# iamycy/golf

Hardware: AMD Instinct MI355X
Metric: audio samples/sec (24 kHz) GOLF-ss synth, batch=32x2 s, 4 batches in flight (higher is better)
Workload: dtype f32

## Files before the change

### golf_amd/csrc/glottal_osc.hip

```cpp
#include "common.h"
#include "device_common.h"
#include "lpc_p1f.h"
#include <algorithm>

namespace golf {

struct OscGeom {
    int P;
    int N;
    int hop_t;
    int nint;
    int ntile;
    int pre_stride;
    size_t off_cw, off_ttot, off_pre, off_part, off_bfr, off_bf4, off_look, total;
};
#define OSC_SCAN_TILE 1024

static void osc_geom(int B, int Tp, int phase_hop, int Fw, int w_hop, int os, OscGeom* g) {
    g->P = phase_hop * os;
    g->N = g->P > 1 ? (Tp - 1) * g->P + 1 : Tp;
    g->hop_t = w_hop * os;
    g->nint = (int)ceil_div(g->N, g->hop_t);
    size_t o = 0;
    g->ntile = (int)ceil_div(Tp, OSC_SCAN_TILE);
// ... 1640 lines not shown
    if (amp) expect = std::min(expect, amp_hop > 1 ? (Fa - 1) * amp_hop + 1 : Fa);
    if (tscale) expect = std::min(expect, ts_hop > 1 ? (Fs - 1) * ts_hop + 1 : Fs);
    if (hp.poff) expect = (int)std::min<int64_t>(expect, (int64_t)(hp.Fo - 1) * hp.po_hop + 1);
    if (Tout != expect) return fail(GOLF_EINVAL, "%s: Tout=%d, expected %d", who, Tout, expect);
    if (amp && dyn_lds && (size_t)(g.nrows + 1) * H * sizeof(float) > 60 * 1024)
        return fail(GOLF_EUNSUPPORTED, "%s: amplitude hop %d too fine for %d harmonics (LDS staging); pass amplitudes "
                    "at a coarser hop or fold them into tscale/hscale", who, amp_hop, H);
    if (dyn_lds && HARM_STATIC_LDS + dyn_lds > HARM_LDS_LIMIT) {
        if (amp)
            return fail(GOLF_EUNSUPPORTED, "%s: amplitude hop %d too fine for %d harmonics%s (LDS staging: %zu bytes, limit "
                        "%zu); pass amplitudes at a coarser hop or fold them into tscale/hscale", who, amp_hop, H,
                        hp.phi0 ? " with initial_phase" : "", HARM_STATIC_LDS + dyn_lds, HARM_LDS_LIMIT);
        return fail(GOLF_EUNSUPPORTED, "%s: %d harmonics%s too many for the LDS staging (%zu bytes, limit %zu)", who, H,
                    hp.phi0 ? " with initial_phase" : "", HARM_STATIC_LDS + dyn_lds, HARM_LDS_LIMIT);
    }
    return GOLF_OK;
}

struct SrcArgs {
    const float* phase; int64_t phase_stride; OscLook look; u64* Ttot; const float* wsel; int Fw; const float* table; int n_tab, L,
        lshift, Tp, hop_t; const float* Bf4; float* out; int64_t out_stride; int Tout, dmin, nrows; const float* addend;
    int64_t addend_stride; int Tadd, B, ntile;
};
struct MapArgs { const float* a; float* PhiT; int F, M, hop, L, NP, nq; float* pmax; unsigned* fixcnt; int B; float* Phi; };
#ifdef SRCMAPS_TIMING
__device__ unsigned long long g_srcmaps_rt[4 * 2048];
extern "C" int golf_debug_srcmaps_rt(unsigned long long* host_out, int n) {
    return (int)hipMemcpyFromSymbol(host_out, HIP_SYMBOL(g_srcmaps_rt), sizeof(unsigned long long) * (size_t)n);
}
#define SRCMAPS_RT(i, v) do { if ((threadIdx.x & 63) == 0 && blockIdx.x < 2048 && (threadIdx.x == 0 || (i) == 3)) g_srcmaps_rt[4 * blockIdx.x + (i)] = (v); } while (0)
#else
#define SRCMAPS_RT(i, v) do { } while (0)
#endif
template <int EE, int KS, int W, int NT>
__global__ __launch_bounds__(512) __attribute__((amdgpu_waves_per_eu(3, 3))) void source_maps_kernel(SrcArgs o, MapArgs m,
                                                                                                     int nblk_f) {
    extern __shared__ __attribute__((aligned(16))) float smem[];
    SRCMAPS_RT(0, __builtin_amdgcn_s_memrealtime());
    SRCMAPS_RT(2, ((unsigned long long)__builtin_amdgcn_s_getreg(4 | (31 << 11))) | ((unsigned long long)(__builtin_amdgcn_s_getreg(20 | (3 << 11)) & 15) << 32));
    if ((int)blockIdx.x < nblk_f) {
        if (threadIdx.x >= 64 * P1F_WPB) return;
#ifndef SRCMAPS_PRIO_MAPS
#define SRCMAPS_PRIO_MAPS 0
#endif
        __builtin_amdgcn_s_setprio(SRCMAPS_PRIO_MAPS);
        p1f_body<W, NT>(m.a, m.PhiT, m.F, m.M, m.hop, m.L, m.NP, m.nq, smem, (int)blockIdx.x, m.pmax, m.fixcnt, m.B, m.Phi);
        SRCMAPS_RT(1, __builtin_amdgcn_s_memrealtime());
    } else {
#ifndef SRCMAPS_PRIO_OSC
#define SRCMAPS_PRIO_OSC 1
#endif
        const int u = (int)blockIdx.x - nblk_f;
#ifdef SRCMAPS_HI_UNITS
        if (u < SRCMAPS_HI_UNITS) __builtin_amdgcn_s_setprio(3); else __builtin_amdgcn_s_setprio(SRCMAPS_PRIO_OSC);
#else
        __builtin_amdgcn_s_setprio(SRCMAPS_PRIO_OSC);
#endif
        const int tile = u / o.B, b = u - tile * o.B;
        osc_fused2_tile<EE, KS, 2048, 512>(o.phase, o.phase_stride, o.look, o.Ttot, o.wsel, o.Fw, o.table, o.n_tab, o.L, o.lshift,
                                           o.Tp, o.hop_t, o.Bf4, o.out, o.out_stride, o.Tout, o.dmin, o.nrows, o.addend,
                                           o.addend_stride, o.Tadd, smem, tile, b, o.ntile);
        SRCMAPS_RT(1, __builtin_amdgcn_s_memrealtime());
    }
}

}

using namespace golf;

// ... 169 lines not shown
                                              addend_stride, Tadd, tap_frags))
            return rc;
        return golf_ltv_allpole_transitions_f32(a, B, T, F, M, hop, ss_ws, ss_ws_bytes, ss_flags, stream);
    }
    hipStream_t st = (hipStream_t)stream;
    const float* Bf4 = tap_frags ? (const float*)tap_frags + kTapFragFloats : (const float*)((char*)osc_ws + g.off_bf4);
    if (!tap_frags) {
        hipLaunchKernelGGL(osc_tap_frags_kernel, dim3(4), dim3(256), 0, st, taps, K, f2.dmin, f2.dmax, f2.KS,
                           (float*)((char*)osc_ws + g.off_bf4), (float*)((char*)osc_ws + g.off_bfr));
        GOLF_LAUNCH_CHECK();
    }
    SrcArgs o;
    o.phase = phase; o.phase_stride = phase_stride;
    o.look.gen = (unsigned*)((char*)osc_ws + g.off_look);
    o.look.ent = (unsigned long long*)((char*)osc_ws + g.off_look + 256 * ceil_div((size_t)B * 4, 256));
    o.Ttot = (u64*)((char*)osc_ws + g.off_ttot);
    o.wsel = wsel; o.Fw = Fw; o.table = table; o.n_tab = n_tab; o.L = L; o.lshift = f2.lshift; o.Tp = Tp; o.hop_t = g.hop_t;
    o.Bf4 = Bf4; o.out = out; o.out_stride = out_stride; o.Tout = Tout; o.dmin = f2.dmin; o.nrows = f2.nrows;
    o.addend = addend; o.addend_stride = addend_stride; o.Tadd = Tadd; o.B = B; o.ntile = f2.ntile_f;
    char* sw = (char*)ss_ws;
    MapArgs m;
    m.a = a; m.PhiT = (float*)(sw + p.off_phiT); m.F = F; m.M = M; m.hop = hop; m.L = p.L; m.NP = p.NP; m.nq = B * p.NP;
    m.pmax = (float*)(sw + p.off_pmax); m.fixcnt = (unsigned*)(sw + p.off_fixcnt); m.B = B;
    m.Phi = (ss_flags & GOLF_SS_TRAINING) ? (float*)(sw + p.off_phi) : (float*)nullptr;
    const int nblk_f = (int)ceil_div(m.nq, P1fGeom<24, 22, 2>::CPW * P1F_WPB);
    const unsigned grid = (unsigned)(nblk_f + B * f2.ntile_f);
#define GOLF_SRC_MAPS(EE, KSV)                                                                                        \
    do {                                                                                                              \
        static const hipError_t lds_attr = hipFuncSetAttribute(                                                       \
            (const void*)source_maps_kernel<EE, KSV, 24, 22>, hipFuncAttributeMaxDynamicSharedMemorySize, 160 * 1024); \
        if (lds_attr != hipSuccess)                                                                                   \
            return fail((int)lds_attr, "source_transitions: cannot raise the dynamic LDS limit: %s",                  \
                        hipGetErrorString(lds_attr));                                                                 \
        hipLaunchKernelGGL((source_maps_kernel<EE, KSV, 24, 22>), dim3(grid), dim3(512), f2.lds, st, o, m, nblk_f);   \
    } while (0)
    if (f2.KS == 12) { if (equal_energy & 1) GOLF_SRC_MAPS(1, 12); else GOLF_SRC_MAPS(0, 12); }
    else             { if (equal_energy & 1) GOLF_SRC_MAPS(1, 16); else GOLF_SRC_MAPS(0, 16); }
#undef GOLF_SRC_MAPS
    GOLF_LAUNCH_CHECK();
    return GOLF_OK;
}

extern "C" int golf_glottal_osc_bwd_wsel_f32(const float* g_out, int64_t g_out_stride, const float* phase,
                                             int64_t phase_stride, int Tp, int phase_hop, const float* wsel, int Fw,
                                             int w_hop, const float* table, int n_tab, int L, int os, int equal_energy,
                                             const float* taps, int K, float* g_wsel, int B, int Tout, void* ws,
// ... 574 lines not shown
```

### golf_amd/csrc/lpc_p1f.h

```cpp
#pragma once
#include "device_common.h"

namespace golf {

typedef float f32x2 __attribute__((ext_vector_type(2)));

constexpr int P1F_WPB = 4;
template <int W, int NT, int NR = 2>
struct P1fGeom {
    static constexpr int KT = 2 * NR;
    static constexpr int NG = (NT + KT - 1) / KT;
    static constexpr int CPW = 64 / NG;
    static constexpr int WAVE_TILE = 64;
    static constexpr int TILE_FLOATS = P1F_WPB * WAVE_TILE;
};
template <int W, int NT, int NR = 2>
__device__ __forceinline__ void p1f_body(const float* __restrict__ a, float* __restrict__ PhiT, int F, int M, int hop,
                                         int L, int NP, int nq, float* __restrict__ tile_all, int blk_id,
                                         float* __restrict__ pmax, unsigned* __restrict__ fixcnt = nullptr, int B = 0,
                                         float* __restrict__ Phi = nullptr) {
    using G = P1fGeom<W, NT, NR>;
    constexpr int KT = G::KT, NG = G::NG, CPW = G::CPW;
    constexpr int NP2 = NT / 2;
    const int lane = threadIdx.x & 63;
    const int wv = __builtin_amdgcn_readfirstlane(threadIdx.x >> 6);
    float* tile = tile_all + wv * G::WAVE_TILE;
    const int cl = lane / NG, grp = lane - cl * NG;
    const int q0 = (blk_id * P1F_WPB + wv) * CPW;
    if (fixcnt && blk_id == 0 && wv == 0)
        for (int e = lane; e < 5 * B + 1; e += 64) fixcnt[e] = 0u;
    if (q0 >= nq) return;
    const int q = q0 + cl;
    const bool live = cl < CPW && q < nq;
    const int jb = KT * grp;
    const int qq = live ? q : (nq - 1);
    const int b = qq / NP, c = qq - b * NP;
    f32x2 h[NR][W];
#pragma unroll
    for (int r = 0; r < NR; ++r)
#pragma unroll
        for (int k = 0; k < W; ++k) {
            const int j = W - 1 - k, j0 = jb + 2 * r;
            h[r][k] = f32x2{(j == j0 && j0 < M) ? 1.f : 0.f, (j == j0 + 1 && j0 + 1 < M) ? 1.f : 0.f};
        }
    f32x2 a0p[NP2], ddp[NP2];
    const float inv_hop = 1.0f / (float)hop;
    int fcur = -1;
    const int nblk = L / W;
    for (int blk = 0; blk < nblk; ++blk) {
        const int t0 = c * L + blk * W;
        const int f = t0 / hop;
        if (f != fcur) {
            fcur = f;
// ... 107 lines not shown
```

### golf_amd/csrc/lpc_ss.hip

```cpp
#include "common.h"
#include "device_common.h"
#include "lpc_p1f.h"
#include <cstdlib>
#include <type_traits>

namespace golf {

static float phi_guard() {
    static const float v = [] { const char* e = getenv("GOLF_SS_PHI_GUARD"); return e ? (float)atof(e) : 30.f; }();
    return v;
}
static float phi_guard2() {
    static const float v = [] { const char* e = getenv("GOLF_SS_PHI_GUARD2"); return e ? (float)atof(e) : 8.f; }();
    return v;
}
static float group_log2_guard() {
    static const float v = [] { const char* e = getenv("GOLF_SS_GROUP_LOG2"); return e ? (float)atof(e) : 96.f; }();
    return v;
}
static int hot_all_16ths() {
    static const int v = [] { const char* e = getenv("GOLF_SS_HOT_ALL_16THS"); return e ? atoi(e) : 16; }();
    return v;
}
static int hot_count() {
// ... 531 lines not shown
            }
            const R cf0 = cfq[(NT - 1) % PD];
            const int sp = (s - 1 + W) % W;
#pragma unroll
            for (int r = 0; r < KT; ++r) h[r][s] = __builtin_elementwise_fma(-cf0, h[r][sp], -(ra[r] + rb[r]));
            __builtin_amdgcn_sched_barrier(0);
        }
    }
#pragma unroll
    for (int r = 0; r < KT; ++r) {
        const int j = jb + r;
        if (j < NT) {
            float* o = Phi + ((size_t)q * NT + j) * W;
#pragma unroll
            for (int i = 0; i < W; ++i) o[i] = (i < M && j < M) ? (float)h[r][W - 1 - i] : 0.f;
        }
    }
}

template <int W, int NT, int NR = 2>
__global__ __launch_bounds__(64 * P1F_WPB) void lpc_p1f_kernel(const float* __restrict__ a, float* __restrict__ PhiT,
                                                               int F, int M, int hop, int L, int NP, int nq,
                                                               float* __restrict__ pmax, unsigned* __restrict__ fixcnt,
                                                               int B, float* __restrict__ Phi) {
    __shared__ __attribute__((aligned(16))) float tile_all[P1fGeom<W, NT, NR>::TILE_FLOATS];
    p1f_body<W, NT, NR>(a, PhiT, F, M, hop, L, NP, nq, tile_all, blockIdx.x, pmax, fixcnt, B, Phi);
}

template <int W, int NT>
__device__ __forceinline__ void p1z_units(const float* __restrict__ ex, int64_t ex_stride,
                                          const float* __restrict__ gain, const float* __restrict__ a,
                                          float* __restrict__ z, int T, int F, int M, int hop, int L, int NP, int ncg,
                                          int B, int upw, int zblk, float (*xt)[Tile<W, 16>::SIZE]) {
    const int wv = __builtin_amdgcn_readfirstlane(threadIdx.x >> 6);
    light_wave_priority();
    for (int u = 0; u < upw; ++u) {
        const int unit = (zblk * 4 + wv) * upw + u;
        if (unit >= ncg * B) return;
        fwdq_body<W, NT, 0>(ex, ex_stride, gain, a, nullptr, z, 0, T, F, M, hop, L, NP, NP, nullptr, xt[wv], nullptr,
                            unit / ncg, unit - (unit / ncg) * ncg, threadIdx.x & 63);
        wave_lds_fence();
    }
}

template <int W, int NT>
__global__ __launch_bounds__(64 * P1F_WPB) void lpc_p1fz_kernel(const float* __restrict__ ex, int64_t ex_stride,
                                                                const float* __restrict__ gain,
                                                                const float* __restrict__ a, float* __restrict__ z,
                                                                float* __restrict__ PhiT, int T, int F, int M, int hop,
                                                                int L, int NP, int nq, int nblk_f, int ncg, int B,
                                                                int upw, float* __restrict__ pmax,
                                                                unsigned* __restrict__ fixcnt, float* __restrict__ Phi) {
    using TL = Tile<W, 16>;
    __shared__ __attribute__((aligned(16))) float tile_all[P1fGeom<W, NT>::TILE_FLOATS];
    __shared__ float xt[P1F_WPB][TL::SIZE];
    if ((int)blockIdx.x < nblk_f) {
        p1f_body<W, NT>(a, PhiT, F, M, hop, L, NP, nq, tile_all, blockIdx.x, pmax, fixcnt, B, Phi);
    } else {
        p1z_units<W, NT>(ex, ex_stride, gain, a, z, T, F, M, hop, L, NP, ncg, B, upw, (int)blockIdx.x - nblk_f, xt);
    }
}

template <int W, int NT, int KT>
__global__ __launch_bounds__(256) void lpc_p1hz_kernel(const float* __restrict__ ex, int64_t ex_stride,
                                                       const float* __restrict__ gain, const float* __restrict__ a,
                                                       float* __restrict__ z, float* __restrict__ Phi,
                                                       float* __restrict__ PhiT, int T, int F, int M, int hop, int L,
                                                       int NP, int nq, int nblk_h, int ncg, int B, int upw) {
    using TL = Tile<W, 16>;
    __shared__ float xt[4][TL::SIZE];
    if ((int)blockIdx.x < nblk_h) {
        constexpr int NG = (NT + KT - 1) / KT;
        const int nqb = (nq + 63) / 64;
        const int unit = blockIdx.x * 4 + __builtin_amdgcn_readfirstlane(threadIdx.x >> 6);
        const int qblk = unit / NG, grp = unit - qblk * NG;
        if (qblk >= nqb) return;
        p1_hom_body<W, NT, KT, double>(qblk, grp, a, Phi, PhiT, F, M, hop, L, NP, nq);
    } else {
        p1z_units<W, NT>(ex, ex_stride, gain, a, z, T, F, M, hop, L, NP, ncg, B, upw, (int)blockIdx.x - nblk_h, xt);
    }
}

template <int W, int NT>
__global__ __launch_bounds__(256) void lpc_transpose_kernel(const float* __restrict__ Phi, float* __restrict__ PhiT,
                                                            int nq, float* __restrict__ pmax,
                                                            unsigned* __restrict__ fixcnt, int B) {
    __shared__ float t[4][NT * (W + 1)];
    const int wv = threadIdx.x >> 6, lane = threadIdx.x & 63;
    if (fixcnt && blockIdx.x == 0)
        for (int e = threadIdx.x; e < 5 * B + 1; e += 256) fixcnt[e] = 0u;
    const int q = blockIdx.x * 4 + wv;
    if (q >= nq) return;
    const float* src = Phi + (size_t)q * NT * W;
    float* dst = PhiT + (size_t)q * NT * W;
    float* tt = t[wv];
    unsigned mx = 0u;
    for (int e = lane; e < NT * W; e += 64) {
        const int j = e / W, i = e - j * W;
        const float v = src[e];
        tt[j * (W + 1) + i] = v;
        mx = max(mx, __float_as_uint(fabsf(v)));
    }
    if (pmax) {
#pragma unroll
        for (int off = 32; off >= 1; off >>= 1) mx = max(mx, (unsigned)__shfl_xor((int)mx, off));
        if (lane == 0) pmax[q] = __uint_as_float(mx);
    }
    __builtin_amdgcn_s_waitcnt(0);
    __builtin_amdgcn_wave_barrier();
    for (int e = lane; e < NT * W; e += 64) {
        const int i = e / W, j = e - i * W;
        dst[e] = (j < NT) ? tt[j * (W + 1) + i] : 0.f;
    }
// ... 40 lines not shown
        if (g3 > 0.f && hot16 > 0 && n * 16u >= (unsigned)NP * (unsigned)hot16) d.t3 = true;
        else if (d.t2) d.nhot = n;
    }
    if (d.t3) d.nhot = (unsigned)NP;
    return d;
}

template <int CTRL>
__device__ __forceinline__ double dppd(double v) {
    const long long x = __builtin_bit_cast(long long, v);
    const unsigned lo = (unsigned)__builtin_amdgcn_update_dpp(0, (int)(unsigned)x, CTRL, 0xF, 0xF, true);
    const unsigned hi = (unsigned)__builtin_amdgcn_update_dpp(0, (int)(unsigned)(x >> 32), CTRL, 0xF, 0xF, true);
    return __builtin_bit_cast(double, ((long long)hi << 32) | (long long)lo);
}
struct FixArgs {
    const float* a;
    float* PhiT;
    float* Phi;
    double* Phi64;
    const float* pmax;
    unsigned* tier;
    unsigned* status;
    unsigned* fixcnt;
    int F, M, hop, L, NP, B;
    float g1, g2, g3, glog;
    int hot16, hotn;
    int accurate;
};

constexpr int kHotListMax = 512;
template <typename T> __device__ __forceinline__ void st_through(T* p, T v) {
    __hip_atomic_store(p, v, __ATOMIC_RELAXED, __HIP_MEMORY_SCOPE_AGENT);
}
template <int W, int NT>
__device__ __forceinline__ void fixup_wave(const FixArgs& fa, int b, bool writes_tier, unsigned short* __restrict__ hotlist) {
    constexpr int TPL = quad_tpl(W, NT);
    const int lane = threadIdx.x & 63;
    const int row = lane >> 2, r = lane & 3;
    const int NP = fa.NP, M = fa.M, F = fa.F, hop = fa.hop, L = fa.L;
    const float* pm = fa.pmax + (size_t)b * NP;
    const UttTier d = utterance_tier(pm, NP, lane, fa.g1, fa.g2, fa.g3, fa.accurate, fa.glog, fa.hot16, fa.hotn);
    if (writes_tier && lane == 0) {
        fa.tier[2 * b] = d.t3 ? kTierPrecise : (d.t2 ? kTierHot : 0u);
        fa.tier[2 * b + 1] = d.nhot;
    }
    if (d.nhot == 0u) return;
    const bool listed = NP <= kHotListMax;
    if (listed) {
        int base = 0;
        for (int c0 = 0; c0 < NP; c0 += 64) {
            const int c = c0 + lane;
            const bool h = c < NP && (d.t3 || !(fabsf(pm[c < NP ? c : 0]) <= fa.g2));
            const unsigned long long m = __builtin_amdgcn_ballot_w64(h);
            const int pre = __builtin_amdgcn_mbcnt_hi((unsigned)(m >> 32), __builtin_amdgcn_mbcnt_lo((unsigned)m, 0u));
            if (h) hotlist[base + pre] = (unsigned short)c;
            base += __builtin_popcountll(m);
        }
        wave_lds_fence();
    }
    const int total = (listed ? (int)d.nhot : NP) * NT;
    unsigned done = 0u;
    for (;;) {
        int k0 = 0;
        if (lane == 0) k0 = (int)atomicAdd(fa.fixcnt + fa.B + b, 16u);
        k0 = __builtin_amdgcn_readfirstlane(k0);
        if (k0 >= total) break;
        const int k = k0 + row;
        const bool live = k < total;
        done += (unsigned)((total - k0 < 16) ? total - k0 : 16);
        const int h = live ? k / NT : 0, j = live ? k - h * NT : 0;
        const int c = listed ? (int)hotlist[h] : h;
        const bool hot = live && (listed || d.t3 || !(fabsf(pm[c]) <= fa.g2));
        if (!hot) continue;
        const size_t q = (size_t)b * NP + c;
        double* o64 = fa.Phi64 + (q * NT + j) * W;
        if (d.t3)
            for (int i = 4 * TPL + r; i < W; i += 4) st_through(o64 + i, 0.0);
        if (j >= M) {
            if (d.t3) {
#pragma unroll
                for (int kk = 0; kk < TPL; ++kk) st_through(o64 + r * TPL + kk, 0.0);
            }
            continue;
// ... 58 lines not shown
            if (fa.Phi) {
                float* o2 = fa.Phi + (q * NT + j) * W;
#pragma unroll
                for (int kk = 0; kk < TPL; ++kk) {
                    const int i = r * TPL + kk;
                    if (i < W) st_through(o2 + i, i < M ? (float)w[TPL - 1 - kk] : 0.f);
                }
            }
        }
        if (d.t3) {
#pragma unroll
            for (int kk = 0; kk < TPL; ++kk) {
                const int i = r * TPL + kk;
                st_through(o64 + i, i < M ? w[TPL - 1 - kk] : 0.0);
            }
        }
    }
    if (!done) return;
    __builtin_amdgcn_fence(__ATOMIC_RELEASE, "workgroup");
    __builtin_amdgcn_s_waitcnt(0x0F70);
    if (lane == 0 && done) atomicAdd(fa.fixcnt + b, done);
}

__device__ __forceinline__ void wait_for_fixup(const FixArgs& fa, int b, unsigned nhot, int NT) {
    const unsigned expected = (fa.NP <= kHotListMax ? nhot : (unsigned)fa.NP) * (unsigned)NT;
    unsigned it = 0u;
    while (__hip_atomic_load(fa.fixcnt + b, __ATOMIC_RELAXED, __HIP_MEMORY_SCOPE_AGENT) < expected) {
        __builtin_amdgcn_s_sleep(8);
        if (++it > (1u << 16)) {
            if ((threadIdx.x & 63) == 0) atomicOr(fa.fixcnt + 2 * fa.B, 1u);
            break;
        }
    }
    __builtin_amdgcn_fence(__ATOMIC_ACQUIRE, "agent");
}

template <int W, int NT>
__global__ __launch_bounds__(256) void lpc_fixup_kernel(FixArgs fa) {
    __shared__ unsigned short hotlist[4][kHotListMax];
    const int wv = __builtin_amdgcn_readfirstlane(threadIdx.x >> 6);
    fixup_wave<W, NT>(fa, blockIdx.y, blockIdx.x == 0 && wv == 0, hotlist[wv]);
}

__device__ __forceinline__ double lane_bcast_d(double v, int lane) {
    const long long x = __builtin_bit_cast(long long, v);
    const unsigned lo = (unsigned)__builtin_amdgcn_readlane((int)(unsigned)x, lane);
    const unsigned hi = (unsigned)__builtin_amdgcn_readlane((int)(unsigned)(x >> 32), lane);
    return __builtin_bit_cast(double, ((long long)hi << 32) | (long long)lo);
}

template <int W, int NT>
__device__ __forceinline__ void precise_fwd_scan_w1(const double* __restrict__ P64, const float* __restrict__ zb,
                                                    float* __restrict__ Sb, int sstride, int NP, int lane) {
    const bool act = lane < NT;
    const int ii = act ? lane : 0;
    constexpr int D = 4;
    double buf[D][NT];
    float zc[D];
    auto fetch = [&](int u, int c) {
        const int cl = c < NP ? c : NP - 1;
        const double* mp = P64 + (size_t)cl * NT * W + ii;
#pragma unroll
        for (int j = 0; j < NT; ++j) buf[u][j] = mp[(size_t)j * W];
        zc[u] = zb[(size_t)cl * W + ii];
// ... 658 lines not shown
    static constexpr int BYTES = HOT + (COMP > ZP ? COMP : ZP);
};
template <int W, int NT>
__global__ __launch_bounds__(256) void lpc_group_prepass_kernel(const float* __restrict__ PhiT,
                                                                float* __restrict__ z, float* __restrict__ MT,
                                                                float* __restrict__ V, int NP, int NG, int B,
                                                                int parts, FixArgs fa, int KF1, int KF2,
                                                                float* __restrict__ MTt, ZPassArgs zp) {
    using PL = PrepassLds<W, NT>;
    using TL = Tile<W, 16>;
    __shared__ __attribute__((aligned(32))) unsigned char lds_raw[PL::BYTES];
    unsigned short (*hot_lds)[kHotListMax] = reinterpret_cast<unsigned short (*)[kHotListMax]>(lds_raw);
    double* pb_lds = reinterpret_cast<double*>(lds_raw + PL::HOT);
    light_wave_priority();
    if (zp.gflag && blockIdx.x == 0) {
        for (int i = threadIdx.x; i < zp.ngflag; i += 256) zp.gflag[i] = 0u;
        if (threadIdx.x == 0 && zp.nonfinite) zp.nonfinite[0] = 0u;
    }
    const bool fix = fa.pmax != nullptr && (parts & 1);
    const int nu = NG * B;
    const int nf1 = fix ? B * KF1 : 0, nz = (parts & 2) ? (nu + 3) / 4 : 0, nc = (parts & 1) ? nu : 0;
    int blk = (int)blockIdx.x;
    const int wv = __builtin_amdgcn_readfirstlane(threadIdx.x >> 6), lane = threadIdx.x & 63;
    if (blk < nf1) {
        fixup_wave<W, NT>(fa, blk / KF1, blk % KF1 == 0 && wv == 0, hot_lds[wv]);
        return;
    }
    blk -= nf1;
    if (blk >= nz + nc) {
        blk -= nz + nc;
        if (fix) fixup_wave<W, NT>(fa, blk / KF2, false, hot_lds[wv]);
        return;
    }
    const bool comp = blk >= nz;
    int b, g;
    float* zl = nullptr;
    if (comp) {
        blk -= nz;
        if (blk % NG == NG - 1 && NP % kGroup != 0 && !MTt) return;
        b = blk / NG; g = blk % NG;
    } else {
        const int u2 = blk * 4 + wv;
        if (u2 >= nu) return;
        b = u2 / NG; g = u2 % NG;
        if (parts & 4) {
            float* xt = reinterpret_cast<float*>(lds_raw + PL::HOT) + wv * (TL::SIZE + kGroup * 32);
            zl = xt + TL::SIZE;
            fwdq_body<W, NT, 0>(zp.ex, zp.ex_stride, zp.gain, fa.a, nullptr, z, 0, zp.T, fa.F, fa.M, fa.hop, fa.L, NP, NP,
                                nullptr, xt, nullptr, b, g, lane, nullptr, zl);
            wave_lds_fence();
        }
    }
    if (fa.pmax) {
        const int c = g * kGroup + (lane & 15);
        const float v = c < NP ? fabsf(fa.pmax[(size_t)b * NP + c]) : 0.f;
        if (__builtin_amdgcn_ballot_w64(!(v <= fa.g2)) != 0ull) {
            const UttTier d = utterance_tier(fa.pmax + (size_t)b * NP, NP, lane, fa.g1, fa.g2, fa.g3, fa.accurate, fa.glog, fa.hot16, fa.hotn);
            if (d.t3) {
                if (fix) fixup_wave<W, NT>(fa, b, false, hot_lds[wv]);
                return;
            }
            if (d.nhot > 0u && !fa.accurate) {
                fixup_wave<W, NT>(fa, b, false, hot_lds[wv]);
                wait_for_fixup(fa, b, d.nhot, NT);
            }
        }
    }
    if (comp)    group_composite_wg<W, NT>(PhiT, MT, NP, NG, b, g, pb_lds, MTt);
    else if (zl) group_scan_lds<W, NT>(PhiT, zl, V, b, g, NP, NG, lane);
    else         group_zscan_body<W, NT>(PhiT, z, V, NP, NG, b, g, lane);
}

#ifdef FWDQ2_TIMING
__device__ unsigned long long g_fq_stamps[2 * 64 * 64 * 8];
#define FQ_STAMP(p, i) do { if ((p) && threadIdx.x == 0) (p)[i] = __builtin_amdgcn_s_memtime(); } while (0)
extern "C" int golf_debug_fwdq2_stamps(unsigned long long* host_out, int n) {
    return (int)hipMemcpyFromSymbol(host_out, HIP_SYMBOL(g_fq_stamps), sizeof(unsigned long long) * (size_t)n, 0, hipMemcpyDeviceToHost);
}
#else
#define FQ_STAMP(p, i) do { } while (0)
#endif

struct NoWait { __device__ __forceinline__ void operator()() const {} };
template <int W, int NT, bool THIN = false, bool SAMEK = false, typename PRE = NoWait, int MAPIO = 0>
__device__ __forceinline__ void group_prologue(const float* __restrict__ PhiT, const float* __restrict__ MT,
                                               const float* V, const float* x,
                                               float* __restrict__ st, int b, int g, int NP, int NG, int lane,
                                               unsigned long long* fqs = nullptr, PRE pre = PRE(), float* mapl = nullptr) {
// ... 1032 lines not shown
static int device_cu_count() {
    constexpr int kMaxDev = 16;
    static int cache[kMaxDev] = {};
    int dev = 0;
    if (hipGetDevice(&dev) != hipSuccess || dev < 0 || dev >= kMaxDev) return 256;
    if (cache[dev] == 0) {
        int n = 0;
        if (hipDeviceGetAttribute(&n, hipDeviceAttributeMultiprocessorCount, dev) != hipSuccess || n < 1) n = 256;
        cache[dev] = n;
    }
    return cache[dev];
}

static FixArgs fix_args(const SsPlan& p, const SsChain& c, const float* a, int B, int F, int M, int hop, char* ws) {
    FixArgs fa;
    fa.a = a;
    fa.PhiT = (float*)(ws + p.off_phiT);
    fa.Phi = (c.training && c.fast) ? (float*)(ws + p.off_phi) : nullptr;
    fa.Phi64 = (double*)(ws + p.off_phi64);
    fa.pmax = (const float*)(ws + p.off_pmax);
    fa.tier = (unsigned*)(ws + p.off_tier);
    fa.status = (unsigned*)(ws + p.off_status);
    fa.fixcnt = (unsigned*)(ws + p.off_fixcnt);
    fa.F = F; fa.M = M; fa.hop = hop; fa.L = p.L; fa.NP = p.NP;
    fa.B = B;
    fa.g1 = phi_guard(); fa.g2 = phi_guard2(); fa.g3 = phi_guard3(); fa.glog = group_log2_guard();
    fa.hot16 = hot_all_16ths();
    fa.hotn = hot_count();
    fa.accurate = c.fast ? 0 : 1;
    return fa;
}

template <int W, int NT>
static int launch_fixup(const SsPlan& p, const SsChain& c, const float* a, int B, int F, int M, int hop, char* ws,
                        hipStream_t st) {
    hipLaunchKernelGGL((lpc_fixup_kernel<W, NT>), dim3((unsigned)(c.k1 + c.k2), B), dim3(256), 0, st,
                       fix_args(p, c, a, B, F, M, hop, ws));
    GOLF_LAUNCH_CHECK();
    return GOLF_OK;
}

template <int W, int NT>
static int launch_composites(const SsPlan& p, const SsChain& c, const float* a, int B, int F, int M, int hop, char* ws,
                             hipStream_t st) {
    if constexpr (NT <= 24) {
        if (c.two_level) {
            hipLaunchKernelGGL((lpc_group_prepass_kernel<W, NT>), dim3((unsigned)(c.nf + c.nu)), dim3(256), 0, st,
                               (const float*)(ws + p.off_phiT), (float*)nullptr, (float*)(ws + p.off_mt),
                               (float*)nullptr, p.NP, p.NG, B, 1, fix_args(p, c, a, B, F, M, hop, ws), c.k1, c.k2,
                               c.training ? (float*)(ws + p.off_mtT) : (float*)nullptr, ZPassArgs{nullptr, 0, nullptr, 0});
            GOLF_LAUNCH_CHECK();
            return GOLF_OK;
        }
    }
    return launch_fixup<W, NT>(p, c, a, B, F, M, hop, ws, st);
}

template <int W, int NT>
static int launch_maps(const SsPlan& p, const float* a, int B, int F, int M, int hop, char* ws, bool training, hipStream_t st) {
    float* Phi = (float*)(ws + p.off_phi);
    float* PhiT = (float*)(ws + p.off_phiT);
    const int nq = B * p.NP;
    hipLaunchKernelGGL((lpc_p1f_kernel<W, NT, 2>), dim3((unsigned)ceil_div(nq, P1fGeom<W, NT, 2>::CPW * P1F_WPB)),
                       dim3(64 * P1F_WPB), 0, st, a, PhiT, F, M, hop, p.L, p.NP, nq, (float*)(ws + p.off_pmax),
                       (unsigned*)(ws + p.off_fixcnt), B, training ? Phi : (float*)nullptr);
    GOLF_LAUNCH_CHECK();
    return GOLF_OK;
}

template <int W, int NT>
static int launch_transitions(const SsPlan& p, const SsChain& c, bool composites, const float* a, int B, int F, int M,
                              int hop, char* ws, hipStream_t st) {
    if (p.NP <= 0) return GOLF_OK;
    if (c.fast) {
        if (int rc = launch_maps<W, NT>(p, a, B, F, M, hop, ws, c.training, st)) return rc;
        if (!composites) return GOLF_OK;
        return launch_composites<W, NT>(p, c, a, B, F, M, hop, ws, st);
    }
    float* Phi = (float*)(ws + p.off_phi);
    float* PhiT = (float*)(ws + p.off_phiT);
    const int nq = B * p.NP;
    constexpr int NG = (NT + 2) / 3;
    hipLaunchKernelGGL((lpc_p1h_kernel<W, NT, 3, double>), dim3((unsigned)ceil_div(ceil_div(nq, 64) * NG, 4)),
                       dim3(256), 0, st, a, Phi, PhiT, F, M, hop, p.L, p.NP, nq);
    GOLF_LAUNCH_CHECK();
    hipLaunchKernelGGL((lpc_transpose_kernel<W, NT>), dim3((unsigned)ceil_div(nq, 4)), dim3(256), 0, st,
                       (const float*)Phi, PhiT, nq, (float*)(ws + p.off_pmax), (unsigned*)(ws + p.off_fixcnt), B);
    GOLF_LAUNCH_CHECK();
    return composites ? launch_composites<W, NT>(p, c, a, B, F, M, hop, ws, st) : GOLF_OK;
}

struct ForkJoin {
    static hipEvent_t next_event() {
        constexpr int kMaxDev = 16;
        static thread_local hipEvent_t ring[kMaxDev][64] = {};
        static thread_local unsigned head[kMaxDev] = {};
        int dev = 0;
        if (hipGetDevice(&dev) != hipSuccess || dev < 0 || dev >= kMaxDev) return nullptr;
        hipEvent_t& e = ring[dev][head[dev]++ & 63];
        if (!e && hipEventCreateWithFlags(&e, hipEventDisableTiming) != hipSuccess) return nullptr;
        return e;
    }
    int record_and_wait(hipStream_t from, hipStream_t to) {
        hipEvent_t ev = next_event();
        if (!ev) return 1;
        if (hipEventRecord(ev, from) != hipSuccess) return 1;
        if (hipStreamWaitEvent(to, ev, 0) != hipSuccess) return 1;
        return 0;
    }
};
// ... 4 lines not shown
                      hipStream_t side, hipStream_t st) {
    float* PhiT = (float*)(ws + p.off_phiT);
    float* z = (float*)(ws + p.off_z);
    float* S = (float*)(ws + p.off_S);
    const unsigned* tier = p.NP > 0 ? (const unsigned*)(ws + p.off_tier) : nullptr;
    unsigned* nonfinite = (unsigned*)(ws + p.off_status);
    const double* Phi64 = (const double*)(ws + p.off_phi64);
    constexpr int D = 8;
    ForkJoin fork, join;
    switch (c.maps) {
        case SsMaps::Own:
            if (int rc = launch_maps<W, NT>(p, a, B, F, M, hop, ws, c.training, st)) return rc;
            break;
        case SsMaps::WithZeroState: {
            constexpr int KT = 3;
            const int nq = B * p.NP, ncg = (int)ceil_div(p.NP, 16);
            const int64_t nunit = (int64_t)ncg * B;
            const int nblk = c.fast ? (int)ceil_div(nq, P1fGeom<W, NT>::CPW * P1F_WPB) : (int)ceil_div(ceil_div(nq, 64) * ((NT + KT - 1) / KT), 4);
            const int upw = ss_upw(nblk, nunit, n_cu), nblk_z = (int)ceil_div(nunit, 4 * upw);
            if (c.fast) {
                hipLaunchKernelGGL((lpc_p1fz_kernel<W, NT>), dim3((unsigned)(nblk + nblk_z)), dim3(64 * P1F_WPB),
                                   0, st, ex, ex_stride, gain, a, z, PhiT, T, F, M, hop, p.L, p.NP, nq, nblk, ncg,
                                   B, upw, (float*)(ws + p.off_pmax), (unsigned*)(ws + p.off_fixcnt),
                                   c.training ? (float*)(ws + p.off_phi) : (float*)nullptr);
                GOLF_LAUNCH_CHECK();
            } else {
                float* Phi = (float*)(ws + p.off_phi);
                hipLaunchKernelGGL((lpc_p1hz_kernel<W, NT, KT>), dim3((unsigned)(nblk + nblk_z)), dim3(256), 0, st,
                                   ex, ex_stride, gain, a, z, Phi, PhiT, T, F, M, hop, p.L, p.NP, nq, nblk, ncg, B,
                                   upw);
                GOLF_LAUNCH_CHECK();
                hipLaunchKernelGGL((lpc_transpose_kernel<W, NT>), dim3((unsigned)ceil_div(nq, 4)), dim3(256), 0, st,
                                   (const float*)Phi, PhiT, nq, (float*)(ws + p.off_pmax),
                                   (unsigned*)(ws + p.off_fixcnt), B);
                GOLF_LAUNCH_CHECK();
            }
            break;
        }
        case SsMaps::ViaTransitions:
            if (c.fork && fork.record_and_wait(st, side)) return fail((int)hipErrorUnknown, "ltv_allpole_fwd: stream fork failed");
            if (int rc = launch_transitions<W, NT>(p, c, true, a, B, F, M, hop, ws, c.fork ? side : st)) return rc;
            break;
        default: break;
    }
    if (c.zero_state == SsZeroState::Own) {
        hipLaunchKernelGGL((lpc_fwdq_kernel<W, NT, 0>), dim3((unsigned)ceil_div(p.NP, 16), B), dim3(64), 0, st, ex,
                           ex_stride, gain, a, (const float*)nullptr, z, (int64_t)0, T, F, M, hop, p.L, p.NP, p.NP,
                           (const float*)nullptr, (const unsigned*)nullptr);
        GOLF_LAUNCH_CHECK();
    }
    if (c.join && join.record_and_wait(side, st)) return fail((int)hipErrorUnknown, "ltv_allpole_fwd: stream join failed");
    if constexpr (NT <= 24) {
        if (c.two_level) {
            float* MT = (float*)(ws + p.off_mt);
            float* Vz = (float*)(ws + p.off_gv);
            float* Vd = Vz + (size_t)B * p.NG * 32;
            float* dfc = (float*)(ws + p.off_z2);
// ... 358 lines not shown
```

### golf_amd/csrc/lpc_ss_plan.h

```cpp
#pragma once
#include <cstddef>
#include <cstdint>

#include "golf_amd.h"

namespace golf {

inline int64_t ceil_div(int64_t a, int64_t b) { return (a + b - 1) / b; }
inline size_t align_up(size_t x, size_t a) { return (x + a - 1) / a * a; }

struct SsPlan {
    int W;
    int NT;
    int L;
    int NC;
    int NP;
    int seg;
    int NSEG;
    bool serial;
    int NG, GS;
    size_t off_phi, off_phiT, off_z, off_E, off_z2, off_S, off_zadj, off_lam, off_g, off_pa, off_pg, off_mt, off_gv, off_pmax, total;
    size_t off_tier, off_S1, off_status, off_phi64, off_fixcnt;
    size_t off_m64, off_v64, off_g64;
    size_t off_mtT, off_L1, off_wadj, off_dadj;
// ... 81 lines not shown
    p->NG = 0;
    p->GS = 0;
    p->off_mt = p->off_gv = o;
    if (p->NP >= 48 && p->NT <= 24) {
        p->GS = 16;
        p->NG = (int)ceil_div(p->NP, p->GS);
        p->off_mt = o;   o = align_up(o + sizeof(float) * (size_t)B * p->NG * p->NT * W, 256);
        p->off_gv = o; o = align_up(o + sizeof(float) * (size_t)B * p->NG * 32 * 2, 256);
    }
    p->off_S1 = o;   o = align_up(o + sizeof(float) * (size_t)B * p->NC * 32, 256);
    p->off_mtT = o;  o = align_up(o + sizeof(float) * (size_t)B * (p->NG > 0 ? p->NG : 1) * p->NT * W, 256);
    p->off_L1 = o;   o = align_up(o + sizeof(float) * (size_t)B * (p->NC + 1) * 32, 256);
    p->off_wadj = o; o = align_up(o + sizeof(float) * (size_t)B * (p->NG > 0 ? p->NG : 1) * 32 * 2, 256);
    p->off_dadj = o; o = align_up(o + sizeof(float) * (size_t)B * p->NC * W, 256);
    p->off_phi64 = o; o = align_up(o + sizeof(double) * (size_t)B * (p->NP > 0 ? p->NP : 1) * p->NT * W, 256);
    p->off_m64 = o;  o = align_up(o + sizeof(double) * (size_t)B * (p->NG > 0 ? p->NG : 1) * p->NT * W, 256);
    p->off_v64 = o;  o = align_up(o + sizeof(double) * (size_t)B * (p->NG > 0 ? p->NG : 1) * 32, 256);
    p->off_g64 = o;  o = align_up(o + sizeof(double) * (size_t)B * (p->NG + 1) * 32, 256);
    p->off_gflag = o; o = align_up(o + sizeof(unsigned) * (size_t)B * (p->NG + 1), 256);
    p->total = o;
    return true;
}

inline bool ss_has_maps(const SsPlan& p) { return p.W > 0 && !p.serial && p.NP > 0; }

#ifndef GOLF_SS_TWO_LEVEL_WAVES
#define GOLF_SS_TWO_LEVEL_WAVES 0
#endif
inline bool ss_two_level(const SsPlan& p, int B, int flags, int n_cu) {
    const int64_t cap = GOLF_SS_TWO_LEVEL_WAVES > 0 ? (int64_t)GOLF_SS_TWO_LEVEL_WAVES : (int64_t)2 * n_cu;
    return p.NG > 0 && !(flags & GOLF_SS_FLAT_SCAN) && (int64_t)B * p.NG <= cap;
}

enum class SsMaps {
    None,
    Have,
    Own,
    WithZeroState,
    ViaTransitions,
};
enum class SsZeroState { None, WithMaps, InPrepass, Own };
enum class SsOwed { None, Prepass, Fixup };
struct SsChain {
    bool fast;
    bool training;
    bool two_level;
// ... 70 lines not shown
```

Measured before the change: 22.38 billion.

## Publish per-utterance fixup tier and hot list once; let idle waves steal fixup work

A lead wave now computes the utterance tier and hot-column list once and publishes them to global memory behind a ready flag. Other waves read the flag instead of recomputing utterance_tier and rebuilding the hot list. The ready flags are zeroed alongside fixcnt in the map kernels. Spare fixup waves also scan the ready flags of other utterances and claim their outstanding fixup units, balancing load across utterances. This adds atomic loads, fences and reuse of the off_E workspace region, which could race with or alias other data.

```diff
diff --git a/golf_amd/csrc/glottal_osc.hip b/golf_amd/csrc/glottal_osc.hip
--- a/golf_amd/csrc/glottal_osc.hip
+++ b/golf_amd/csrc/glottal_osc.hip
@@ -1686,7 +1686,7 @@
         lshift, Tp, hop_t; const float* Bf4; float* out; int64_t out_stride; int Tout, dmin, nrows; const float* addend;
     int64_t addend_stride; int Tadd, B, ntile;
 };
-struct MapArgs { const float* a; float* PhiT; int F, M, hop, L, NP, nq; float* pmax; unsigned* fixcnt; int B; float* Phi; };
+struct MapArgs { const float* a; float* PhiT; int F, M, hop, L, NP, nq; float* pmax; unsigned* fixcnt; int B; float* Phi; unsigned* ready; };
 #ifdef SRCMAPS_TIMING
 __device__ unsigned long long g_srcmaps_rt[4 * 2048];
 extern "C" int golf_debug_srcmaps_rt(unsigned long long* host_out, int n) {
@@ -1708,7 +1708,7 @@
 #define SRCMAPS_PRIO_MAPS 0
 #endif
         __builtin_amdgcn_s_setprio(SRCMAPS_PRIO_MAPS);
-        p1f_body<W, NT>(m.a, m.PhiT, m.F, m.M, m.hop, m.L, m.NP, m.nq, smem, (int)blockIdx.x, m.pmax, m.fixcnt, m.B, m.Phi);
+        p1f_body<W, NT>(m.a, m.PhiT, m.F, m.M, m.hop, m.L, m.NP, m.nq, smem, (int)blockIdx.x, m.pmax, m.fixcnt, m.B, m.Phi, m.ready);
         SRCMAPS_RT(1, __builtin_amdgcn_s_memrealtime());
     } else {
 #ifndef SRCMAPS_PRIO_OSC
@@ -1924,6 +1924,7 @@
     MapArgs m;
     m.a = a; m.PhiT = (float*)(sw + p.off_phiT); m.F = F; m.M = M; m.hop = hop; m.L = p.L; m.NP = p.NP; m.nq = B * p.NP;
     m.pmax = (float*)(sw + p.off_pmax); m.fixcnt = (unsigned*)(sw + p.off_fixcnt); m.B = B;
+    m.ready = (unsigned*)(sw + ss_off_ready(p));
     m.Phi = (ss_flags & GOLF_SS_TRAINING) ? (float*)(sw + p.off_phi) : (float*)nullptr;
     const int nblk_f = (int)ceil_div(m.nq, P1fGeom<24, 22, 2>::CPW * P1F_WPB);
     const unsigned grid = (unsigned)(nblk_f + B * f2.ntile_f);
diff --git a/golf_amd/csrc/lpc_p1f.h b/golf_amd/csrc/lpc_p1f.h
--- a/golf_amd/csrc/lpc_p1f.h
+++ b/golf_amd/csrc/lpc_p1f.h
@@ -18,7 +18,7 @@
 __device__ __forceinline__ void p1f_body(const float* __restrict__ a, float* __restrict__ PhiT, int F, int M, int hop,
                                          int L, int NP, int nq, float* __restrict__ tile_all, int blk_id,
                                          float* __restrict__ pmax, unsigned* __restrict__ fixcnt = nullptr, int B = 0,
-                                         float* __restrict__ Phi = nullptr) {
+                                         float* __restrict__ Phi = nullptr, unsigned* __restrict__ ready = nullptr) {
     using G = P1fGeom<W, NT, NR>;
     constexpr int KT = G::KT, NG = G::NG, CPW = G::CPW;
     constexpr int NP2 = NT / 2;
@@ -27,8 +27,10 @@
     float* tile = tile_all + wv * G::WAVE_TILE;
     const int cl = lane / NG, grp = lane - cl * NG;
     const int q0 = (blk_id * P1F_WPB + wv) * CPW;
-    if (fixcnt && blk_id == 0 && wv == 0)
+    if (fixcnt && blk_id == 0 && wv == 0) {
         for (int e = lane; e < 5 * B + 1; e += 64) fixcnt[e] = 0u;
+        for (int e = lane; e < B; e += 64) ready[e] = 0u;
+    }
     if (q0 >= nq) return;
     const int q = q0 + cl;
     const bool live = cl < CPW && q < nq;
diff --git a/golf_amd/csrc/lpc_ss.hip b/golf_amd/csrc/lpc_ss.hip
--- a/golf_amd/csrc/lpc_ss.hip
+++ b/golf_amd/csrc/lpc_ss.hip
@@ -577,9 +577,9 @@
 __global__ __launch_bounds__(64 * P1F_WPB) void lpc_p1f_kernel(const float* __restrict__ a, float* __restrict__ PhiT,
                                                                int F, int M, int hop, int L, int NP, int nq,
                                                                float* __restrict__ pmax, unsigned* __restrict__ fixcnt,
-                                                               int B, float* __restrict__ Phi) {
+                                                               int B, float* __restrict__ Phi, unsigned* __restrict__ ready) {
     __shared__ __attribute__((aligned(16))) float tile_all[P1fGeom<W, NT, NR>::TILE_FLOATS];
-    p1f_body<W, NT, NR>(a, PhiT, F, M, hop, L, NP, nq, tile_all, blockIdx.x, pmax, fixcnt, B, Phi);
+    p1f_body<W, NT, NR>(a, PhiT, F, M, hop, L, NP, nq, tile_all, blockIdx.x, pmax, fixcnt, B, Phi, ready);
 }
 
 template <int W, int NT>
@@ -605,12 +605,13 @@
                                                                 float* __restrict__ PhiT, int T, int F, int M, int hop,
                                                                 int L, int NP, int nq, int nblk_f, int ncg, int B,
                                                                 int upw, float* __restrict__ pmax,
-                                                                unsigned* __restrict__ fixcnt, float* __restrict__ Phi) {
+                                                                unsigned* __restrict__ fixcnt, float* __restrict__ Phi,
+                                                                unsigned* __restrict__ ready) {
     using TL = Tile<W, 16>;
     __shared__ __attribute__((aligned(16))) float tile_all[P1fGeom<W, NT>::TILE_FLOATS];
     __shared__ float xt[P1F_WPB][TL::SIZE];
     if ((int)blockIdx.x < nblk_f) {
-        p1f_body<W, NT>(a, PhiT, F, M, hop, L, NP, nq, tile_all, blockIdx.x, pmax, fixcnt, B, Phi);
+        p1f_body<W, NT>(a, PhiT, F, M, hop, L, NP, nq, tile_all, blockIdx.x, pmax, fixcnt, B, Phi, ready);
     } else {
         p1z_units<W, NT>(ex, ex_stride, gain, a, z, T, F, M, hop, L, NP, ncg, B, upw, (int)blockIdx.x - nblk_f, xt);
     }
@@ -639,11 +640,14 @@
 template <int W, int NT>
 __global__ __launch_bounds__(256) void lpc_transpose_kernel(const float* __restrict__ Phi, float* __restrict__ PhiT,
                                                             int nq, float* __restrict__ pmax,
-                                                            unsigned* __restrict__ fixcnt, int B) {
+                                                            unsigned* __restrict__ fixcnt, int B,
+                                                            unsigned* __restrict__ ready) {
     __shared__ float t[4][NT * (W + 1)];
     const int wv = threadIdx.x >> 6, lane = threadIdx.x & 63;
-    if (fixcnt && blockIdx.x == 0)
+    if (fixcnt && blockIdx.x == 0) {
         for (int e = threadIdx.x; e < 5 * B + 1; e += 256) fixcnt[e] = 0u;
+        for (int e = threadIdx.x; e < B; e += 256) ready[e] = 0u;
+    }
     const int q = blockIdx.x * 4 + wv;
     if (q >= nq) return;
     const float* src = Phi + (size_t)q * NT * W;
@@ -730,43 +734,123 @@
     unsigned* tier;
     unsigned* status;
     unsigned* fixcnt;
+    unsigned* ready;
+    unsigned* hotpub;
+    int hotwords;
     int F, M, hop, L, NP, B;
     float g1, g2, g3, glog;
     int hot16, hotn;
     int accurate;
 };
 
-constexpr int kHotListMax = 512;
+constexpr int kHotListMax = ss_hot_list_max;
 template <typename T> __device__ __forceinline__ void st_through(T* p, T v) {
     __hip_atomic_store(p, v, __ATOMIC_RELAXED, __HIP_MEMORY_SCOPE_AGENT);
 }
+template <typename T> __device__ __forceinline__ T ld_through(const T* p) {
+    return __hip_atomic_load(p, __ATOMIC_RELAXED, __HIP_MEMORY_SCOPE_AGENT);
+}
+
+constexpr unsigned kPubReady = 0x80000000u, kPubT3 = 0x40000000u, kPubT2 = 0x20000000u, kPubCount = 0x1FFFFFFFu;
+__device__ __forceinline__ unsigned pack_tier(const UttTier& d) {
+    return kPubReady | (d.t3 ? kPubT3 : 0u) | (d.t2 ? kPubT2 : 0u) | (d.nhot & kPubCount);
+}
+__device__ __forceinline__ UttTier unpack_tier(unsigned w) {
+    UttTier d;
+    d.t3 = (w & kPubT3) != 0u; d.t2 = (w & kPubT2) != 0u; d.nhot = w & kPubCount;
+    return d;
+}
+__device__ __forceinline__ int fixup_units(const UttTier& d, int NP, int NT) {
+    return (NP <= kHotListMax ? (int)d.nhot : (d.nhot ? NP : 0)) * NT;
+}
+
+__device__ __forceinline__ void build_hot_list(const FixArgs& fa, const float* __restrict__ pm, const UttTier& d, int lane,
+                                               unsigned short* __restrict__ hotlist) {
+    const int NP = fa.NP;
+    int base = 0;
+    for (int c0 = 0; c0 < NP; c0 += 64) {
+        const int c = c0 + lane;
+        const bool h = c < NP && (d.t3 || !(fabsf(pm[c < NP ? c : 0]) <= fa.g2));
+        const unsigned long long m = __builtin_amdgcn_ballot_w64(h);
+        const int pre = __builtin_amdgcn_mbcnt_hi((unsigned)(m >> 32), __builtin_amdgcn_mbcnt_lo((unsigned)m, 0u));
+        if (h) hotlist[base + pre] = (unsigned short)c;
+        base += __builtin_popcountll(m);
+    }
+    wave_lds_fence();
+}
+
+__device__ __forceinline__ UttTier publish_tier(const FixArgs& fa, int b, int lane, unsigned short* __restrict__ hotlist) {
+    const float* pm = fa.pmax + (size_t)b * fa.NP;
+    const UttTier d = utterance_tier(pm, fa.NP, lane, fa.g1, fa.g2, fa.g3, fa.accurate, fa.glog, fa.hot16, fa.hotn);
+    if (lane == 0) {
+        fa.tier[2 * b] = d.t3 ? kTierPrecise : (d.t2 ? kTierHot : 0u);
+        fa.tier[2 * b + 1] = d.nhot;
+    }
+    if (d.nhot != 0u && fa.NP <= kHotListMax) {
+        build_hot_list(fa, pm, d, lane, hotlist);
+        if (!d.t3) {
+            unsigned* g = fa.hotpub + (size_t)b * fa.hotwords;
+            const int nw = ((int)d.nhot + 1) >> 1;
+            for (int i = lane; i < nw; i += 64)
+                st_through(g + i, (unsigned)hotlist[2 * i] | ((unsigned)hotlist[2 * i + 1 < kHotListMax ? 2 * i + 1 : 0] << 16));
+            __builtin_amdgcn_fence(__ATOMIC_RELEASE, "workgroup");
+            __builtin_amdgcn_s_waitcnt(0x0F70);
+        }
+    }
+    if (lane == 0) st_through(fa.ready + b, pack_tier(d));
+    return d;
+}
+
+__device__ __forceinline__ void fetch_hot_list(const FixArgs& fa, int b, const UttTier& d, int lane,
+                                               unsigned short* __restrict__ hotlist) {
+    if (d.nhot == 0u || fa.NP > kHotListMax) return;
+    wave_lds_fence();
+    if (d.t3) {
+        for (int c = lane; c < fa.NP; c += 64) hotlist[c] = (unsigned short)c;
+    } else {
+        const unsigned* g = fa.hotpub + (size_t)b * fa.hotwords;
+        const int nw = ((int)d.nhot + 1) >> 1;
+        constexpr int NL = kHotListMax / 2 / 64;
+        unsigned v[NL];
+#pragma unroll
+        for (int k = 0; k < NL; ++k) v[k] = ld_through(g + (lane + 64 * k < nw ? lane + 64 * k : 0));
+#pragma unroll
+        for (int k = 0; k < NL; ++k)
+            if (lane + 64 * k < nw) {
+                hotlist[2 * (lane + 64 * k)] = (unsigned short)(v[k] & 0xFFFFu);
+                hotlist[2 * (lane + 64 * k) + 1] = (unsigned short)(v[k] >> 16);
+            }
+    }
+    wave_lds_fence();
+}
+
+__device__ __forceinline__ UttTier read_tier(const FixArgs& fa, int b, int lane, unsigned short* __restrict__ hotlist) {
+    const unsigned w = (unsigned)__builtin_amdgcn_readfirstlane((int)ld_through(fa.ready + b));
+    if (!(w & kPubReady)) {
+        const float* pm = fa.pmax + (size_t)b * fa.NP;
+        const UttTier d = utterance_tier(pm, fa.NP, lane, fa.g1, fa.g2, fa.g3, fa.accurate, fa.glog, fa.hot16, fa.hotn);
+        if (d.nhot != 0u && fa.NP <= kHotListMax) {
+            wave_lds_fence();
+            build_hot_list(fa, pm, d, lane, hotlist);
+        }
+        return d;
+    }
+    __builtin_amdgcn_fence(__ATOMIC_ACQUIRE, "agent");
+    const UttTier d = unpack_tier(w);
+    fetch_hot_list(fa, b, d, lane, hotlist);
+    return d;
+}
+
 template <int W, int NT>
-__device__ __forceinline__ void fixup_wave(const FixArgs& fa, int b, bool writes_tier, unsigned short* __restrict__ hotlist) {
+__device__ __forceinline__ void fixup_claim(const FixArgs& fa, int b, const UttTier& d, const unsigned short* __restrict__ hotlist) {
     constexpr int TPL = quad_tpl(W, NT);
     const int lane = threadIdx.x & 63;
     const int row = lane >> 2, r = lane & 3;
     const int NP = fa.NP, M = fa.M, F = fa.F, hop = fa.hop, L = fa.L;
     const float* pm = fa.pmax + (size_t)b * NP;
-    const UttTier d = utterance_tier(pm, NP, lane, fa.g1, fa.g2, fa.g3, fa.accurate, fa.glog, fa.hot16, fa.hotn);
-    if (writes_tier && lane == 0) {
-        fa.tier[2 * b] = d.t3 ? kTierPrecise : (d.t2 ? kTierHot : 0u);
-        fa.tier[2 * b + 1] = d.nhot;
-    }
     if (d.nhot == 0u) return;
     const bool listed = NP <= kHotListMax;
-    if (listed) {
-        int base = 0;
-        for (int c0 = 0; c0 < NP; c0 += 64) {
-            const int c = c0 + lane;
-            const bool h = c < NP && (d.t3 || !(fabsf(pm[c < NP ? c : 0]) <= fa.g2));
-            const unsigned long long m = __builtin_amdgcn_ballot_w64(h);
-            const int pre = __builtin_amdgcn_mbcnt_hi((unsigned)(m >> 32), __builtin_amdgcn_mbcnt_lo((unsigned)m, 0u));
-            if (h) hotlist[base + pre] = (unsigned short)c;
-            base += __builtin_popcountll(m);
-        }
-        wave_lds_fence();
-    }
-    const int total = (listed ? (int)d.nhot : NP) * NT;
+    const int total = fixup_units(d, NP, NT);
     unsigned done = 0u;
     for (;;) {
         int k0 = 0;
@@ -871,6 +955,51 @@
     if (lane == 0 && done) atomicAdd(fa.fixcnt + b, done);
 }
 
+template <int W, int NT>
+__device__ __forceinline__ void fixup_wave(const FixArgs& fa, int home, bool lead, bool publisher, unsigned short* __restrict__ hotlist,
+                                           int pool = 0) {
+    const int lane = threadIdx.x & 63;
+    const int B = fa.B;
+    UttTier d;
+    d.t2 = d.t3 = false; d.nhot = 0u;
+    const bool own = lead || (__builtin_amdgcn_readfirstlane((int)__hip_atomic_load(fa.ready + home, __ATOMIC_RELAXED,
+                                                                                     __HIP_MEMORY_SCOPE_WORKGROUP)) & (int)kPubReady) == 0;
+    if (publisher) d = publish_tier(fa, home, lane, hotlist);
+    else if (own) {
+        const float* pm = fa.pmax + (size_t)home * fa.NP;
+        d = utterance_tier(pm, fa.NP, lane, fa.g1, fa.g2, fa.g3, fa.accurate, fa.glog, fa.hot16, fa.hotn);
+        if (d.nhot != 0u && fa.NP <= kHotListMax) build_hot_list(fa, pm, d, lane, hotlist);
+    }
+    int b = home, o0 = 0, u = 0;
+    unsigned w = 0u;
+    unsigned long long todo = 0ull;
+    for (;;) {
+        fixup_claim<W, NT>(fa, b, d, hotlist);
+        if (own) return;
+        while (todo == 0ull) {
+            if (o0 >= B) return;
+            const int off = o0 + lane;
+            const bool in = off < B;
+            o0 += 64;
+            u = home + (in ? off : 0);
+            u = u >= B ? u - B : u;
+            w = __hip_atomic_load(fa.ready + u, __ATOMIC_RELAXED, __HIP_MEMORY_SCOPE_WORKGROUP);
+            const UttTier du = unpack_tier(w);
+            const bool hot = in && (w & kPubReady) != 0u && du.nhot != 0u &&
+                             (off == 0 || (unsigned)off * (unsigned)pool * 16u < (unsigned)fixup_units(du, fa.NP, NT));
+            if (__builtin_amdgcn_ballot_w64(hot) == 0ull) continue;
+            const unsigned claimed = ld_through(fa.fixcnt + B + u);
+            todo = __builtin_amdgcn_ballot_w64(hot && claimed < (unsigned)fixup_units(du, fa.NP, NT));
+            __builtin_amdgcn_fence(__ATOMIC_ACQUIRE, "agent");
+        }
+        const int l = __builtin_ctzll(todo);
+        todo &= todo - 1ull;
+        b = __builtin_amdgcn_readlane(u, l);
+        d = unpack_tier((unsigned)__builtin_amdgcn_readlane((int)w, l));
+        fetch_hot_list(fa, b, d, lane, hotlist);
+    }
+}
+
 __device__ __forceinline__ void wait_for_fixup(const FixArgs& fa, int b, unsigned nhot, int NT) {
     const unsigned expected = (fa.NP <= kHotListMax ? nhot : (unsigned)fa.NP) * (unsigned)NT;
     unsigned it = 0u;
@@ -888,7 +1017,7 @@
 __global__ __launch_bounds__(256) void lpc_fixup_kernel(FixArgs fa) {
     __shared__ unsigned short hotlist[4][kHotListMax];
     const int wv = __builtin_amdgcn_readfirstlane(threadIdx.x >> 6);
-    fixup_wave<W, NT>(fa, blockIdx.y, blockIdx.x == 0 && wv == 0, hotlist[wv]);
+    fixup_wave<W, NT>(fa, (int)blockIdx.y, true, blockIdx.x == 0 && wv == 0, hotlist[wv]);
 }
 
 __device__ __forceinline__ double lane_bcast_d(double v, int lane) {
@@ -1593,16 +1722,14 @@
     const int nf1 = fix ? B * KF1 : 0, nz = (parts & 2) ? (nu + 3) / 4 : 0, nc = (parts & 1) ? nu : 0;
     int blk = (int)blockIdx.x;
     const int wv = __builtin_amdgcn_readfirstlane(threadIdx.x >> 6), lane = threadIdx.x & 63;
-    if (blk < nf1) {
-        fixup_wave<W, NT>(fa, blk / KF1, blk % KF1 == 0 && wv == 0, hot_lds[wv]);
+    if (blk < nf1 || blk >= nf1 + nz + nc) {
+        if (!fix) return;
+        const bool lead = blk < nf1;
+        const int k = lead ? blk : blk - (nf1 + nz + nc), KF = lead ? KF1 : KF2;
+        fixup_wave<W, NT>(fa, k / KF, lead, lead && k % KF == 0 && wv == 0, hot_lds[wv], 4 * KF2);
         return;
     }
     blk -= nf1;
-    if (blk >= nz + nc) {
-        blk -= nz + nc;
-        if (fix) fixup_wave<W, NT>(fa, blk / KF2, false, hot_lds[wv]);
-        return;
-    }
     const bool comp = blk >= nz;
     int b, g;
     float* zl = nullptr;
@@ -1626,15 +1753,11 @@
         const int c = g * kGroup + (lane & 15);
         const float v = c < NP ? fabsf(fa.pmax[(size_t)b * NP + c]) : 0.f;
         if (__builtin_amdgcn_ballot_w64(!(v <= fa.g2)) != 0ull) {
-            const UttTier d = utterance_tier(fa.pmax + (size_t)b * NP, NP, lane, fa.g1, fa.g2, fa.g3, fa.accurate, fa.glog, fa.hot16, fa.hotn);
-            if (d.t3) {
-                if (fix) fixup_wave<W, NT>(fa, b, false, hot_lds[wv]);
-                return;
-            }
-            if (d.nhot > 0u && !fa.accurate) {
-                fixup_wave<W, NT>(fa, b, false, hot_lds[wv]);
-                wait_for_fixup(fa, b, d.nhot, NT);
-            }
+            const UttTier d = read_tier(fa, b, lane, hot_lds[wv]);
+            const bool waits = !d.t3 && d.nhot > 0u && !fa.accurate;
+            if ((d.t3 && fix) || waits) fixup_claim<W, NT>(fa, b, d, hot_lds[wv]);
+            if (d.t3) return;
+            if (waits) wait_for_fixup(fa, b, d.nhot, NT);
         }
     }
     if (comp)    group_composite_wg<W, NT>(PhiT, MT, NP, NG, b, g, pb_lds, MTt);
@@ -2713,6 +2836,9 @@
     fa.tier = (unsigned*)(ws + p.off_tier);
     fa.status = (unsigned*)(ws + p.off_status);
     fa.fixcnt = (unsigned*)(ws + p.off_fixcnt);
+    fa.ready = (unsigned*)(ws + ss_off_ready(p));
+    fa.hotpub = (unsigned*)(ws + ss_off_hot(p, B));
+    fa.hotwords = ss_hot_words(p);
     fa.F = F; fa.M = M; fa.hop = hop; fa.L = p.L; fa.NP = p.NP;
     fa.B = B;
     fa.g1 = phi_guard(); fa.g2 = phi_guard2(); fa.g3 = phi_guard3(); fa.glog = group_log2_guard();
@@ -2754,7 +2880,8 @@
     const int nq = B * p.NP;
     hipLaunchKernelGGL((lpc_p1f_kernel<W, NT, 2>), dim3((unsigned)ceil_div(nq, P1fGeom<W, NT, 2>::CPW * P1F_WPB)),
                        dim3(64 * P1F_WPB), 0, st, a, PhiT, F, M, hop, p.L, p.NP, nq, (float*)(ws + p.off_pmax),
-                       (unsigned*)(ws + p.off_fixcnt), B, training ? Phi : (float*)nullptr);
+                       (unsigned*)(ws + p.off_fixcnt), B, training ? Phi : (float*)nullptr,
+                       (unsigned*)(ws + ss_off_ready(p)));
     GOLF_LAUNCH_CHECK();
     return GOLF_OK;
 }
@@ -2776,7 +2903,8 @@
                        dim3(256), 0, st, a, Phi, PhiT, F, M, hop, p.L, p.NP, nq);
     GOLF_LAUNCH_CHECK();
     hipLaunchKernelGGL((lpc_transpose_kernel<W, NT>), dim3((unsigned)ceil_div(nq, 4)), dim3(256), 0, st,
-                       (const float*)Phi, PhiT, nq, (float*)(ws + p.off_pmax), (unsigned*)(ws + p.off_fixcnt), B);
+                       (const float*)Phi, PhiT, nq, (float*)(ws + p.off_pmax), (unsigned*)(ws + p.off_fixcnt), B,
+                       (unsigned*)(ws + ss_off_ready(p)));
     GOLF_LAUNCH_CHECK();
     return composites ? launch_composites<W, NT>(p, c, a, B, F, M, hop, ws, st) : GOLF_OK;
 }
@@ -2827,7 +2955,8 @@
                 hipLaunchKernelGGL((lpc_p1fz_kernel<W, NT>), dim3((unsigned)(nblk + nblk_z)), dim3(64 * P1F_WPB),
                                    0, st, ex, ex_stride, gain, a, z, PhiT, T, F, M, hop, p.L, p.NP, nq, nblk, ncg,
                                    B, upw, (float*)(ws + p.off_pmax), (unsigned*)(ws + p.off_fixcnt),
-                                   c.training ? (float*)(ws + p.off_phi) : (float*)nullptr);
+                                   c.training ? (float*)(ws + p.off_phi) : (float*)nullptr,
+                                   (unsigned*)(ws + ss_off_ready(p)));
                 GOLF_LAUNCH_CHECK();
             } else {
                 float* Phi = (float*)(ws + p.off_phi);
@@ -2837,7 +2966,7 @@
                 GOLF_LAUNCH_CHECK();
                 hipLaunchKernelGGL((lpc_transpose_kernel<W, NT>), dim3((unsigned)ceil_div(nq, 4)), dim3(256), 0, st,
                                    (const float*)Phi, PhiT, nq, (float*)(ws + p.off_pmax),
-                                   (unsigned*)(ws + p.off_fixcnt), B);
+                                   (unsigned*)(ws + p.off_fixcnt), B, (unsigned*)(ws + ss_off_ready(p)));
                 GOLF_LAUNCH_CHECK();
             }
             break;
diff --git a/golf_amd/csrc/lpc_ss_plan.h b/golf_amd/csrc/lpc_ss_plan.h
--- a/golf_amd/csrc/lpc_ss_plan.h
+++ b/golf_amd/csrc/lpc_ss_plan.h
@@ -127,6 +127,11 @@
     return true;
 }
 
+constexpr int ss_hot_list_max = 512;
+inline size_t ss_off_ready(const SsPlan& p) { return p.off_E; }
+inline int ss_hot_words(const SsPlan& p) { return ((p.NP < ss_hot_list_max ? p.NP : ss_hot_list_max) + 1) / 2; }
+inline size_t ss_off_hot(const SsPlan& p, int B) { return p.off_E + sizeof(unsigned) * (size_t)B; }
+
 inline bool ss_has_maps(const SsPlan& p) { return p.W > 0 && !p.serial && p.NP > 0; }
 
 #ifndef GOLF_SS_TWO_LEVEL_WAVES
```

Result: no change. 22.42 billion (median of 4 runs) (+0.2%).
